# happyjin/Gaussian_process

Hardware: AMD Instinct MI355X
Metric: GP-fit+predict sec and achieved fp64 TFLOP/s, N=65536 d=8, 1/2/4/8 MI355X (higher is better)
Workload: dtype f64; 1 GPU; GP fit+predict N=65536 d=8 n_test=4096 (BASELINE configs[2]); N=65536, d=8, n_test=4096, partition=single GPU

## Files before the change

gaussian_process_amd/csrc/driver.hip:

```cpp
#include "gpmi_ctx.h"
#include "gpmi_plan.h"

namespace gpmi {

hipError_t panel_rec(hipStream_t s, double* A, int64_t ld, int64_t mrows, int64_t off, int64_t w,
                     int64_t col_offset, int64_t* info) {
    hipError_t e;
    const bool fused = tuning().panel_fused && w % 128 == 0 && off % 128 == 0;
    const int64_t leaf = fused ? 128 : IB;
    if (w <= leaf) {
        double* Ajj = A + off * ld + off;
        const int64_t below = mrows - off - leaf;
        if (fused) {
            if ((e = launch_potrf128(s, Ajj, ld, col_offset + off, info)) != hipSuccess) return e;
            if (below > 0) return launch_trsm128(s, Ajj, ld, A + (off + leaf) * ld + off, ld, below);
            return hipSuccess;
        }
        if ((e = launch_potf2_64(s, Ajj, ld, col_offset + off, info)) != hipSuccess) return e;
        if (below > 0) return launch_trsm_rlt64(s, Ajj, ld, A + (off + IB) * ld + off, ld, below);
        return hipSuccess;
    }
    const int64_t h = (w / 2) / leaf * leaf;
    if ((e = panel_rec(s, A, ld, mrows, off, h, col_offset, info)) != hipSuccess) return e;
    {
        const int64_t c0 = off + h;
        const int64_t r0 = c0 / TILE * TILE;
        const GemmArgs g = gemm_minus_lower(A + r0 * ld + c0, ld, A + r0 * ld + off, ld, A + c0 * ld + off, ld, mrows - r0,
                                            w - h, h, r0 - c0);
        if ((e = launch_gemm_nt(s, g)) != hipSuccess) return e;
    }
    return panel_rec(s, A, ld, mrows, off + h, w - h, col_offset, info);
}

hipError_t panel_factor(hipStream_t s, double* A, int64_t ld, int64_t nb, int64_t mrows,
                        int64_t col_offset, int64_t* info) {
    return panel_rec(s, A, ld, mrows, 0, nb, col_offset, info);
}

hipError_t trsm_rec(hipStream_t s, const double* L, int64_t ldl, double* X, int64_t ldx, int64_t m,
                    int64_t off, int64_t w) {
    hipError_t e;
    const bool fused = tuning().panel_fused && w % 128 == 0 && off % 128 == 0 && m % 128 == 0;
    const int64_t leaf = fused ? 128 : IB;
    if (w <= leaf) {
        if (fused) return launch_trsm128(s, L + off * ldl + off, ldl, X + off, ldx, m);
        return launch_trsm_rlt64(s, L + off * ldl + off, ldl, X + off, ldx, m);
    }
    const int64_t h = (w / 2) / leaf * leaf;
    if ((e = trsm_rec(s, L, ldl, X, ldx, m, off, h)) != hipSuccess) return e;
    const GemmArgs g = gemm_minus(X + off + h, ldx, X + off, ldx, L + (off + h) * ldl + off, ldl, m, w - h, h);
    if ((e = launch_gemm_nt(s, g)) != hipSuccess) return e;
    return trsm_rec(s, L, ldl, X, ldx, m, off + h, w - h);
}

hipError_t trsm_block(hipStream_t s, const double* L, int64_t ldl, double* X, int64_t ldx,
                      int64_t m, int64_t nb) {
    return trsm_rec(s, L, ldl, X, ldx, m, 0, nb);
}

std::vector<int64_t> block_schedule(const gpmi_ctx* c, int64_t ncols) {
    return plan_block_widths(c->block(ncols), ncols, c->nb == 0, c->ramp);
}

hipError_t cholesky_inplace(gpmi_ctx* c, double* A, int64_t ld, int64_t ncols, int64_t nrows,
                            int64_t* info, bool account, int64_t carried_rows, const SweepFollower* follow) {
    hipError_t e;
    hipStream_t sm = c->stream;
    const std::vector<int64_t> widths = block_schedule(c, ncols);
    const int64_t NB = c->block(ncols);
    const bool la = c->lookahead && c->pstream && ncols > NB && ncols >= c->la_min;
    hipStream_t sp_ = la ? c->pstream : sm;
    const bool large = la && ncols >= 49152;
    const bool slack = large && (c->slack_forms & 1);
    SharingScope shallow((la || follow) ? Sharing::beside_update().with_panel_slack(slack) : sharing());
    const bool col_on_panel = la && (!large || (c->slack_forms & 2));
    const int slot_p = account ? GPMI_T_CHOL_PANEL : GPMI_T_COUNT - 1;
    const int slot_t = account ? GPMI_T_CHOL_TRAIL : GPMI_T_COUNT - 1;
    if (la && (e = c->order(sm, sp_)) != hipSuccess) return e;
    auto trail = [&](hipStream_t st, bool counted, int64_t r0, int64_t c0, int64_t k, int64_t nb, int64_t ncol_upd) -> hipError_t {
        GemmArgs g = gemm_minus_lower(A + r0 * ld + c0, ld, A + r0 * ld + k, ld, A + c0 * ld + k, ld, nrows - r0, ncol_upd,
                                      nb, r0 - c0);
        g.role = counted ? 1 : 0;
        const GemmRoute route = gemm_nt_route(g);
        const bool dma = gemm_kernel_is_dma(route.kernel);
        size_t sp = c->span_begin(counted ? (dma ? slot_t : GPMI_T_COUNT - 1) : slot_p, st);
        hipError_t er = launch_gemm_nt(st, g, route);
        c->span_end(sp, st);
        if (account && dma && counted) {
            c->stage_ms[GPMI_T_TRAIL_LAUNCHES] += 1.0;
            c->stage_ms[GPMI_T_TRAIL_FLOPS] += gemm_nt_algorithmic_flops(g, ncols - r0 + 1 + carried_rows);
        }
        return er;
    };
    int64_t k = 0;
    hipEvent_t ev_b = nullptr;
    for (size_t step = 0; step < widths.size(); ++step) {
        const int64_t nb = widths[step];
        size_t sp = c->span_begin(slot_p, sp_);
        {
            SharingScope panel_forms(!la ? sharing().large_lds()
                                     : (ncols - k >= c->shallow_min ? Sharing::beside_update() : Sharing::chip_shared_only()).with_panel_slack(slack));
            e = panel_factor(sp_, A + k * ld + k, ld, nb, nrows - k, k, info);
        }
        c->span_end(sp, sp_);
        if (e != hipSuccess) return e;
        if (la && (e = c->order(sp_, sm)) != hipSuccess) return e;
        const int64_t r0 = k + nb;
        if (follow) {
            if ((e = c->order(sp_, follow->vs)) != hipSuccess) return e;
            {
                SharingScope solve_forms(follow->m >= 2048 ? Sharing::beside_update() : Sharing::chip_shared_only());
                if ((e = trsm_block(follow->vs, A + k * ld + k, ld, follow->V + k, follow->ldv, follow->m, nb)) != hipSuccess) return e;
            }
            if (r0 < ncols) {
                const GemmArgs g = gemm_minus(follow->V + r0, follow->ldv, follow->V + k, follow->ldv, A + r0 * ld + k, ld,
                                              follow->m, ncols - r0, nb);
                SharingScope update_forms(sharing().with_panel_slack(false));
                if ((e = launch_gemm_nt(follow->vs, g)) != hipSuccess) return e;
            }
        }
        k = r0;
        if (r0 >= ncols) continue;
        if (!la) {
            if ((e = trail(sm, true, r0, r0, r0 - nb, nb, ncols - r0)) != hipSuccess) return e;
            continue;
        }
        const int64_t nbn = widths[step + 1];
        if (!col_on_panel) {
            if ((e = trail(sm, true, r0, r0, r0 - nb, nb, nbn)) != hipSuccess) return e;
            if ((e = c->order(sm, sp_)) != hipSuccess) return e;
            if (r0 + nbn < ncols &&
                (e = trail(sm, true, r0 + nbn, r0 + nbn, r0 - nb, nb, ncols - r0 - nbn)) != hipSuccess) return e;
            continue;
        }
        if (ev_b && (e = hipStreamWaitEvent(sp_, ev_b, 0)) != hipSuccess) return e;
        if ((e = trail(sp_, false, r0, r0, r0 - nb, nb, nbn)) != hipSuccess) return e;
        if (r0 + nbn < ncols) {
            if ((e = trail(sm, true, r0 + nbn, r0 + nbn, r0 - nb, nb, ncols - r0 - nbn)) != hipSuccess) return e;
            ev_b = c->new_event();
            if (!ev_b) return c->ev_error;
            if ((e = hipEventRecord(ev_b, sm)) != hipSuccess) return e;
        }
    }
    return hipSuccess;
}

RbfArgs rbf_cross(const gpmi_ctx* c, const double* A, int64_t nA, const Box& ba, const double* B, int64_t nB, const Box& bb,
                  int64_t row0, int64_t nrows, int64_t ncols, double* out, int64_t ld) {
    RbfArgs r;
    r.A = A; r.B = B;
    r.nA = nA; r.nB = nB; r.d = c->d; r.row0 = row0; r.nrows = nrows; r.ncols = ncols;
    r.coef = c->coef; r.sig2 = c->sig2;
    r.kind = c->kind; r.kp0 = c->kp0; r.kp1 = c->kp1;
    for (int i = 0; i < 11; ++i) r.kpv[i] = c->kpv[i];
    r.diag_add = 0.; r.symmetric = 0;
// ... 224 lines not shown
```

gaussian_process_amd/csrc/gpmi_api.hip:

```cpp
#include "gpmi_ctx.h"

using namespace gpmi;

namespace gpmi {
thread_local std::string g_err;

static thread_local Tuning t_dev_tuning;
static thread_local const Tuning* t_tuning = nullptr;
const Tuning& tuning() { return t_tuning ? *t_tuning : t_dev_tuning; }
TuneScope::TuneScope(const Tuning* t) : prev(t_tuning) { t_tuning = t; }
TuneScope::~TuneScope() { t_tuning = prev; }
static thread_local Sharing t_sharing;
Sharing& sharing() { return t_sharing; }

int ard_rescale_train(gpmi_ctx* c) {
    if (!c->ard()) return GPMI_OK;
    HIP_TRY(c->Xz.ensure((size_t)c->N * c->d * 8));
    HIP_TRY(launch_scale_inputs(c->stream, c->X.as<double>(), c->ard_rdev.as<double>(), c->N, c->d, c->Xz.as<double>()));
    HIP_TRY(hipStreamSynchronize(c->stream));
    box_scale(c->boxX, c->ard_r, c->boxZ);
    return GPMI_OK;
}
int ard_rescale_test(gpmi_ctx* c) {
    if (!c->ard()) return GPMI_OK;
    HIP_TRY(c->Xsz.ensure((size_t)c->n * c->d * 8));
    HIP_TRY(launch_scale_inputs(c->stream, c->Xs.as<double>(), c->ard_rdev.as<double>(), c->n, c->d, c->Xsz.as<double>()));
    HIP_TRY(hipStreamSynchronize(c->stream));
    box_scale(c->boxXs, c->ard_r, c->boxZs);
    return GPMI_OK;
}
}

extern "C" {

int gpmi_abi_version(void) { return GPMI_ABI_VERSION; }
const char* gpmi_last_error(void) { return g_err.c_str(); }

int gpmi_device_count(int* count) {
    if (!count) return fail_arg("gpmi_device_count: null pointer");
    int n = 0;
    hipError_t e = hipGetDeviceCount(&n);
    if (e != hipSuccess) { *count = 0; return fail_runtime(e, "hipGetDeviceCount"); }
    *count = n;
    return GPMI_OK;
}

int gpmi_ctx_create(int device, gpmi_ctx** out) {
    if (!out) return fail_arg("gpmi_ctx_create: null out pointer");
    *out = nullptr;
    int n = 0;
    HIP_TRY(hipGetDeviceCount(&n));
    if (device < 0 || device >= n) return fail_arg("gpmi_ctx_create: no such device");
    HIP_TRY(hipSetDevice(device));
    gpmi_ctx* c = new gpmi_ctx();
    c->device = device;
    int prio_lo = 0, prio_hi = 0;
    (void)hipDeviceGetStreamPriorityRange(&prio_lo, &prio_hi);
    hipError_t e = hipStreamCreateWithPriority(&c->stream, hipStreamNonBlocking, prio_lo);
    if (e != hipSuccess) { delete c; return fail_runtime(e, "hipStreamCreate"); }
    e = hipStreamCreateWithPriority(&c->pstream, hipStreamNonBlocking, prio_hi);
    if (e != hipSuccess) { (void)hipStreamDestroy(c->stream); delete c; return fail_runtime(e, "hipStreamCreate"); }
    const char* env;
    if ((env = getenv("GPMI_NB"))) c->nb = std::max<int64_t>(128, atoll(env) / 128 * 128);
    if ((env = getenv("GPMI_LD_PAD"))) c->ld_pad = std::max<int64_t>(0, atoll(env) / 2 * 2);
    if ((env = getenv("GPMI_LOOKAHEAD"))) c->lookahead = atoi(env) ? 1 : 0;
    if ((env = getenv("GPMI_SLACK_FORMS"))) c->slack_forms = atoi(env) & 3;
    *out = c;
    return GPMI_OK;
}

int gpmi_ctx_destroy(gpmi_ctx* c) {
    if (!c) return GPMI_OK;
    for (gpmi_ctx* l : c->lane_ctx) (void)gpmi_ctx_destroy(l);
    c->lane_ctx.clear();
    (void)hipSetDevice(c->device);
    (void)hipStreamSynchronize(c->stream);
    for (DevBuf* b : {&c->X, &c->y, &c->A, &c->info, &c->red, &c->Xs, &c->V, &c->P, &c->vec, &c->dense,
                       &c->U, &c->Kn, &c->gpart, &c->cov_a, &c->cov_b, &c->cov_out, &c->flag, &c->vside,
                       &c->Xz, &c->Xsz, &c->ard_rdev, &c->gsum, &c->lap, &c->lap_part, &c->lap_out, &c->sm, &c->sm_part, &c->sm_E, &c->sm_B, &c->sm_out, &c->loov, &c->loow,
                       &c->sp_Zraw, &c->sp_Z, &c->sp_L, &c->sp_B, &c->sp_W, &c->sp_q, &c->sp_vec, &c->sp_part, &c->sp_scr, &c->sp_info, &c->sp_pred,
                       &c->sp_g0, &c->sp_g1, &c->sp_g2, &c->sp_gE, &c->sp_gpart, &c->sp_gvec})
        b->release();
    for (auto e : c->ev_pool) (void)hipEventDestroy(e);
    (void)hipStreamDestroy(c->stream);
    (void)hipStreamDestroy(c->pstream);
    if (c->vstream) (void)hipStreamDestroy(c->vstream);
    delete c;
    return GPMI_OK;
}

static int set_tuning_option(Tuning& t, const char* name, int64_t value) {
    if (!strcmp(name, "gemm_small_tiles")) {
        t.gemm_small_tiles = value ? 1 : 0;
    } else if (!strcmp(name, "trsm_wave")) {
        t.trsm_wave = value ? 1 : 0;
    } else if (!strcmp(name, "gemm_small_dma")) {
        t.gemm_small_dma = value ? 1 : 0;
    } else if (!strcmp(name, "gemm_persist")) {
        t.gemm_persist = value ? 1 : 0;
    } else if (!strcmp(name, "gemm_ticket")) {
        if (value < 0 || value > 2) return fail_arg("gemm_ticket must be 0 (off), 1 (trailing updates under lookahead) or 2 (every launch)");
        t.gemm_ticket = (int)value;
    } else if (!strcmp(name, "gemm_balance")) {
        t.gemm_balance = value ? 1 : 0;
    } else if (!strcmp(name, "trsv_vinv")) {
        if (value < 0 || value > 2) return fail_arg("trsv_vinv must be 0 (16 x 16 rounds), 1 (one launch per block) or 2 (one launch)");
        t.trsv_vinv = (int)value;
    } else if (!strcmp(name, "panel_fused")) {
        t.panel_fused = value ? 1 : 0;
    } else if (!strcmp(name, "rbf_blocks")) {
        if (value < 1 || value > (1 << 24)) return fail_arg("rbf_blocks must be in 1..2^24");
        t.rbf_blocks = (int)value;
    } else if (!strcmp(name, "gemm_dma_waves")) {
        if (value != 4 && value != 8) return fail_arg("gemm_dma_waves must be 4 or 8");
        t.gemm_dma_waves = (int)value;
    } else if (!strcmp(name, "gemm_tall")) {
        if (value < 0 || value > 1) return fail_arg("gemm_tall must be 0 (128 x 128 blocks) or 1 (256 x 128 blocks for large launches)");
        t.gemm_tall = (int)value;
    } else if (!strcmp(name, "tall_min_tiles")) {
        if (value < 0 || value > (1 << 30)) return fail_arg("tall_min_tiles must be in 0..2^30");
        t.tall_min_tiles = (int)value;
    } else if (!strcmp(name, "tall_min_tiles_slack")) {
        if (value < 0 || value > (1 << 30)) return fail_arg("tall_min_tiles_slack must be in 0..2^30");
        t.tall_min_tiles_slack = (int)value;
    } else if (!strcmp(name, "gemm_dma")) {
        t.gemm_use_dma = value ? 1 : 0;
    } else {
        return -1;
    }
    return GPMI_OK;
}

int gpmi_set_option(gpmi_ctx* c, const char* name, int64_t value) {
    if (!c || !name) return fail_arg("gpmi_set_option: null argument");
    if (!strcmp(name, "nb")) {
        if (value != 0 && (value < 128 || value % 128)) return fail_arg("nb must be 0 (auto) or a positive multiple of 128");
        c->nb = value;
    } else if (!strcmp(name, "ld_pad")) {
        if (value < 0 || value % 2) return fail_arg("ld_pad must be even and >= 0");
        c->ld_pad = value;
        c->res.drop_fit();
    } else if (!strcmp(name, "timing")) {
        c->timing = value ? 1 : 0;
    } else if (!strcmp(name, "lookahead")) {
        c->lookahead = value ? 1 : 0;
    } else if (!strcmp(name, "la_min")) {
        if (value < 0) return fail_arg("la_min must be >= 0");
        c->la_min = value;
    } else if (!strcmp(name, "shallow_min")) {
        if (value < 0) return fail_arg("shallow_min must be >= 0");
        c->shallow_min = value;
    } else if (!strcmp(name, "slack_forms")) {
        if (value < 0 || value > 3) return fail_arg("slack_forms: bit 0 the lower bar of the 256 x 128 form, bit 1 the next block column on the panel stream");
        c->slack_forms = (int)value;
    } else if (!strcmp(name, "one_pass_form")) {
        if (value < 0 || value > 2) return fail_arg("one_pass_form must be 0 (by size), 1 (rows ride) or 2 (rows follow)");
        c->one_pass_form = (int)value;
    } else if (!strcmp(name, "sparse_slab")) {
        if (value < 0) return fail_arg("sparse_slab must be >= 0 (0: by size)");
        c->sparse_slab = value;
    } else if (!strcmp(name, "lanes")) {
        if (value < 0 || value > 8) return fail_arg("lanes must be 0 (by size) .. 8");
        c->lanes = (int)value;
    } else if (!strcmp(name, "ramp")) {
        if (value < 0 || (value & 8) || (value >> 4) > 64) return fail_arg("ramp: bits 0-2 and a tail count of at most 64 in bits 4..");
        c->ramp = (int)value;
    } else {
        const int rc = set_tuning_option(c->tune, name, value);
        if (rc < 0) return fail_arg("gpmi_set_option: unknown option");
        return rc;
    }
    return GPMI_OK;
}

int gpmi_dev_set_option(const char* name, int64_t value) {
    if (!name) return fail_arg("gpmi_dev_set_option: null argument");
    const int rc = set_tuning_option(t_dev_tuning, name, value);
    if (rc < 0) return fail_arg("gpmi_dev_set_option: unknown option");
    return rc;
}

int gpmi_set_kernel(gpmi_ctx* c, int kind, double p0, double p1) {
    if (!c) return fail_arg("gpmi_set_kernel: null context");
    if (kind < 0 || kind == 3 || kind > 6)
        return fail_arg("gpmi_set_kernel: kind must be 0 (rbf), 1 (linear), 2 (periodic) or 4, 5, 6 (Matern nu = 1/2, 3/2, 5/2)");
    if (kind == 2 && (!(p0 != 0.0) || !(p1 != 0.0))) return fail_arg("gpmi_set_kernel: period and lengthscale must be non-zero");
    c->kind = kind; c->kp0 = p0; c->kp1 = p1;
    c->res.drop_fit();
    return GPMI_OK;
}

int gpmi_set_kernel_params(gpmi_ctx* c, int kind, const double* params, int nparams) {
    if (!c || !params) return fail_arg("gpmi_set_kernel_params: null argument");
    if (kind != 3) {
        if (kind < 0 || kind > 6 || nparams != 2) return fail_arg("gpmi_set_kernel_params: kinds 0-2 and 4-6 take 2 parameters");
        return gpmi_set_kernel(c, kind, params[0], params[1]);
    }
    if (nparams != 11) return fail_arg("gpmi_set_kernel_params: the CO2 composite kernel takes 11 hyper-parameters (CO2_example.py:86-89)");
    if (!(params[1] != 0.0) || !(params[3] != 0.0) || !(params[4] != 0.0) || !(params[6] != 0.0) || !(params[7] != 0.0) ||
        !(params[9] != 0.0))
        return fail_arg("gpmi_set_kernel_params: theta_2, 4, 5, 7, 8, 10 divide and must be non-zero");
    c->kind = 3;
    for (int i = 0; i < 11; ++i) c->kpv[i] = params[i];
    c->res.drop_fit();
    return GPMI_OK;
}

int gpmi_sync(gpmi_ctx* c) {
    if (!c) return fail_arg("gpmi_sync: null context");
    HIP_TRY(hipSetDevice(c->device));
    HIP_TRY(hipStreamSynchronize(c->stream));
    return GPMI_OK;
}

static int cov_impl(gpmi_ctx* c, int kind, const double* a, int64_t N, const double* b, int64_t M, int64_t d,
                    double p0, double p1, const double* kpv, double* out);

int gpmi_cov(gpmi_ctx* c, int kind, const double* a, int64_t N, const double* b, int64_t M, int64_t d,
             double p0, double p1, double* out) {
    if (kind < 0 || kind == 3 || kind > 6) return fail_arg("gpmi_cov: kind must be 0, 1, 2, 4, 5 or 6");
    return cov_impl(c, kind, a, N, b, M, d, p0, p1, nullptr, out);
}

int gpmi_cov_params(gpmi_ctx* c, int kind, const double* a, int64_t N, const double* b, int64_t M, int64_t d,
                    const double* params, int nparams, double* out) {
    if (!params) return fail_arg("gpmi_cov_params: null parameters");
    if (kind != 3) {
        if (kind < 0 || kind > 6 || nparams != 2) return fail_arg("gpmi_cov_params: kinds 0-2 and 4-6 take 2 parameters");
        return cov_impl(c, kind, a, N, b, M, d, params[0], params[1], nullptr, out);
    }
    if (nparams != 11) return fail_arg("gpmi_cov_params: the CO2 composite kernel takes 11 hyper-parameters");
    if (!(params[1] != 0.0) || !(params[3] != 0.0) || !(params[4] != 0.0) || !(params[6] != 0.0) || !(params[7] != 0.0) ||
        !(params[9] != 0.0))
        return fail_arg("gpmi_cov_params: theta_2, 4, 5, 7, 8, 10 divide and must be non-zero");
    return cov_impl(c, 3, a, N, b, M, d, 0., 0., params, out);
}

// ... 185 lines not shown

int gpmi_fit_predict_resident(gpmi_ctx* c, double sigma, double ell, double noise_var, double* lml, int64_t* bad_pivot,
                              double* mu, double* out2, int want_sd) {
    if (!c) return fail_arg("gpmi_fit_predict: null context");
    if (!c->res.have_test) return fail_arg("gpmi_fit_predict: no test set (call gpmi_set_test)");
    HIP_TRY(hipSetDevice(c->device));
    TuneScope tune_scope(&c->tune);
    return factorize_impl(c, sigma, ell, noise_var, lml, bad_pivot, true, mu, out2, want_sd);
}

int gpmi_fit_predict_sample_resident(gpmi_ctx* c, double sigma, double ell, double noise_var, double jitter, double* lml,
                                     int64_t* bad_pivot, double* mu, double* out2, int want_sd, double* L_out) {
    if (!c) return fail_arg("gpmi_fit_predict_sample: null context");
    if (!c->res.have_test) return fail_arg("gpmi_fit_predict_sample: no test set (call gpmi_set_test)");
    HIP_TRY(hipSetDevice(c->device));
    TuneScope tune_scope(&c->tune);
    int rc = factorize_impl(c, sigma, ell, noise_var, lml, bad_pivot, true, mu, out2, want_sd, true, jitter);
    if (rc || !L_out) return rc;
    return gpmi_post_chol(c, jitter, L_out, bad_pivot);
}

int gpmi_predict(gpmi_ctx* c, const double* Xs, int64_t n, double* mu, double* out2, int want_sd) {
    int rc = gpmi_set_test(c, Xs, n);
    if (rc) return rc;
    return gpmi_predict_resident(c, mu, out2, want_sd);
}

int gpmi_lml_grad(gpmi_ctx* c, double* d_ell, double* d_sigma) {
    if (!c || !d_ell || !d_sigma) return fail_arg("gpmi_lml_grad: null argument");
    HIP_TRY(hipSetDevice(c->device));
    const Tuning tn = resident_tuning(c);
    TuneScope tune_scope(&tn);
    return lml_grad_impl(c, d_ell, d_sigma);
}

int gpmi_lml_grad_ard(gpmi_ctx* c, double* d_r, double* d_ell, double* d_sigma, double* d_noise) {
    if (!c) return fail_arg("gpmi_lml_grad_ard: null context");
    HIP_TRY(hipSetDevice(c->device));
    const Tuning tn = resident_tuning(c);
    TuneScope tune_scope(&tn);
    return lml_grad_ard_impl(c, d_r, d_ell, d_sigma, d_noise);
}

int gpmi_loo(gpmi_ctx* c, double* mu, double* var, double* logp, double* loo) {
    if (!c) return fail_arg("gpmi_loo: null context");
    HIP_TRY(hipSetDevice(c->device));
    const Tuning tn = resident_tuning(c);
    TuneScope tune_scope(&tn);
    return loo_impl(c, mu, var, logp, loo);
}

int gpmi_loo_grad(gpmi_ctx* c, double* d_ell, double* d_sigma, double* d_noise) {
    if (!c) return fail_arg("gpmi_loo_grad: null context");
    HIP_TRY(hipSetDevice(c->device));
    const Tuning tn = resident_tuning(c);
    TuneScope tune_scope(&tn);
    return loo_grad_impl(c, d_ell, d_sigma, d_noise);
}

int gpmi_grad_trace(gpmi_ctx* c, const double* a_in, const double* b_in, int64_t N, int64_t d, double sigma,
                    double ell, const double* alpha_in, const double* Kinv_in, double* d_ell, double* d_sigma) {
    if (!c || !a_in || !b_in || !alpha_in || !Kinv_in || !d_ell || !d_sigma) return fail_arg("gpmi_grad_trace: null argument");
    HIP_TRY(hipSetDevice(c->device));
    return grad_trace_impl(c, a_in, b_in, N, d, sigma, ell, alpha_in, Kinv_in, d_ell, d_sigma);
}

int gpmi_post_chol(gpmi_ctx* c, double jitter, double* L_out, int64_t* bad_pivot) {
    if (!c || !L_out) return fail_arg("gpmi_post_chol: null argument");
    HIP_TRY(hipSetDevice(c->device));
    TuneScope tune_scope(&c->tune);
    return post_chol_impl(c, jitter, L_out, bad_pivot);
}

int gpmi_post_sample(gpmi_ctx* c, double jitter, const double* Z, int64_t num_fun, double* LZ_out, int64_t* bad_pivot) {
    if (!c || !Z || !LZ_out) return fail_arg("gpmi_post_sample: null argument");
    HIP_TRY(hipSetDevice(c->device));
    TuneScope tune_scope(&c->tune);
    return post_sample_impl(c, jitter, Z, num_fun, LZ_out, bad_pivot);
}

static int lane_prepare(gpmi_ctx* c, gpmi_ctx* l) {
    l->nb = c->nb; l->ld_pad = c->ld_pad; l->lookahead = c->lookahead; l->la_min = c->la_min; l->ramp = c->ramp; l->timing = c->timing;
    l->tune = c->tune;
    l->kind = c->kind; l->kp0 = c->kp0; l->kp1 = c->kp1;
    for (int i = 0; i < 11; ++i) l->kpv[i] = c->kpv[i];
    l->N = c->N; l->d = c->d; l->boxX = c->box_train();
    HIP_TRY(l->X.ensure((size_t)c->N * c->d * 8));
    HIP_TRY(l->y.ensure((size_t)c->N * 8));
    HIP_TRY(hipMemcpyAsync(l->X.p, c->x_train(), (size_t)c->N * c->d * 8, hipMemcpyDeviceToDevice, l->stream));
    HIP_TRY(hipMemcpyAsync(l->y.p, c->y.p, (size_t)c->N * 8, hipMemcpyDeviceToDevice, l->stream));
    HIP_TRY(hipStreamSynchronize(l->stream));
    l->res.drop_train();
    l->res.train_set();
    return GPMI_OK;
}

int gpmi_lml_batch(gpmi_ctx* c, const double* triples, int64_t T, double* lml_out, int* status_out) {
    if (!c || !triples || !lml_out) return fail_arg("gpmi_lml_batch: null argument");
    if (T < 0) return fail_arg("gpmi_lml_batch: T < 0");
    if (!c->res.have_train) return fail_arg("gpmi_lml_batch: no training set (call gpmi_set_train)");
    HIP_TRY(hipSetDevice(c->device));
    const int64_t Np = round_up(c->N, TILE);
    int L = c->lanes ? c->lanes : (Np > 32768 ? 1 : Np >= 24576 ? 3 : Np >= 12288 ? 5 : 4);
    L = (int)std::min<int64_t>(L, std::max<int64_t>(T, 1));
    struct LaMinScope {
        gpmi_ctx* c; int64_t keep;
        ~LaMinScope() { c->la_min = keep; }
    } la_scope{c, c->la_min};
    if (L > 1) c->la_min = std::max<int64_t>(c->la_min, 12288);
    while ((int)c->lane_ctx.size() < L - 1) {
        gpmi_ctx* l = nullptr;
        int rc = gpmi_ctx_create(c->device, &l);
        if (rc) return rc;
        c->lane_ctx.push_back(l);
    }
    for (int j = 0; j < L - 1; ++j) {
        int rc = lane_prepare(c, c->lane_ctx[(size_t)j]);
        if (rc) return rc;
    }
    const int parent_class = (int)((T - 1 + L) % L);
    std::vector<gpmi_ctx*> lane((size_t)L);
    for (int r = 0, nx = 0; r < L; ++r) lane[(size_t)r] = (r == parent_class) ? c : c->lane_ctx[(size_t)nx++];
    std::vector<int> lane_rc((size_t)L, GPMI_OK);
    std::vector<std::string> lane_err((size_t)L);
    std::vector<std::vector<double>> lane_ms((size_t)L, std::vector<double>(GPMI_T_COUNT, 0.0));
    auto work = [&](int r) {
        gpmi_ctx* l = lane[(size_t)r];
        TuneScope tune_scope(&l->tune);
        SharingScope shares_chip(L > 1 ? sharing().and_chip_shared() : sharing());
        if (hipSetDevice(l->device) != hipSuccess) { lane_rc[(size_t)r] = GPMI_ERR_RUNTIME; lane_err[(size_t)r] = "hipSetDevice"; return; }
        for (int64_t t = r; t < T; t += L) {
            const double ell = triples[3 * t], sigma = triples[3 * t + 1], s2 = triples[3 * t + 2];
            double lml = 0.;
            int64_t bad = 0;
            const int rc = factorize_impl(l, sigma, ell, s2, &lml, &bad);
            if (rc == GPMI_ERR_RUNTIME || rc == GPMI_ERR_BAD_ARG) {
                lane_rc[(size_t)r] = rc;
                lane_err[(size_t)r] = g_err;
                return;
            }
            lml_out[t] = lml;
            if (status_out) status_out[t] = rc;
            for (int i = 0; i < GPMI_T_COUNT; ++i) lane_ms[(size_t)r][(size_t)i] += l->stage_ms[i];
        }
    };
    if (L == 1) {
        work(0);
    } else {
        std::vector<std::thread> th;
        for (int r = 0; r < L; ++r) th.emplace_back(work, r);
        for (auto& t : th) t.join();
    }
    for (int r = 0; r < L; ++r)
        if (lane_rc[(size_t)r] != GPMI_OK) {
            g_err = lane_err[(size_t)r];
            return lane_rc[(size_t)r];
        }
    for (int i = 0; i < GPMI_T_COUNT; ++i) {
        c->stage_ms[i] = 0.0;
        for (int r = 0; r < L; ++r) c->stage_ms[i] += lane_ms[(size_t)r][(size_t)i];
    }
    return GPMI_OK;
}

int gpmi_laplace_fit(gpmi_ctx* c, double sigma, double ell, double tol, int max_iter, double* log_q, int* iters,
                     int* converged, double* f_hat) {
    if (!c) return fail_arg("gpmi_laplace_fit: null context");
    HIP_TRY(hipSetDevice(c->device));
    TuneScope tune_scope(&c->tune);
    return laplace_fit_impl(c, sigma, ell, tol, max_iter, log_q, iters, converged, f_hat);
}

int gpmi_laplace_predict_resident(gpmi_ctx* c, double* f_mean, double* f_var, double* prob) {
    if (!c) return fail_arg("gpmi_laplace_predict: null context");
    HIP_TRY(hipSetDevice(c->device));
    return laplace_predict_impl(c, f_mean, f_var, prob);
}

int gpmi_laplace_grad(gpmi_ctx* c, double* d_r, double* d_ell, double* d_sigma) {
    if (!c) return fail_arg("gpmi_laplace_grad: null context");
    HIP_TRY(hipSetDevice(c->device));
    return laplace_grad_impl(c, d_r, d_ell, d_sigma);
}

int gpmi_softmax_fit(gpmi_ctx* c, int n_classes, double sigma, double ell, double tol, int max_iter, double* log_q,
                     int* iters, int* converged, double* f_hat) {
    if (!c) return fail_arg("gpmi_softmax_fit: null context");
    HIP_TRY(hipSetDevice(c->device));
    TuneScope tune_scope(&c->tune);
    return softmax_fit_impl(c, n_classes, sigma, ell, tol, max_iter, log_q, iters, converged, f_hat);
}
// ... 48 lines not shown
```

gaussian_process_amd/csrc/gpmi_ctx.h:

```cpp
#pragma once
#include <algorithm>
#include <cmath>
#include <cstdio>
#include <cstring>
#include <limits>
#include <string>
#include <thread>
#include <vector>

#include "../../include/gpmi.h"
#include "gpmi_internal.h"
#include "gpmi_state.h"

namespace gpmi {

extern thread_local std::string g_err;

inline int fail_runtime(hipError_t e, const char* what) {
    char buf[512];
    snprintf(buf, sizeof buf, "%s: %s (hipError %d)", what, hipGetErrorString(e), (int)e);
    g_err = buf;
    return GPMI_ERR_RUNTIME;
}
inline int fail_arg(const char* what) {
    g_err = what;
    return GPMI_ERR_BAD_ARG;
}

#define HIP_TRY(expr)                                             \
    do {                                                          \
        hipError_t _e = (expr);                                   \
        if (_e != hipSuccess) return fail_runtime(_e, #expr);     \
    } while (0)

inline int64_t round_up(int64_t x, int64_t m) { return (x + m - 1) / m * m; }

struct DevBuf {
    void* p = nullptr;
    size_t cap = 0;
    hipError_t ensure(size_t bytes) {
        if (bytes <= cap) return hipSuccess;
        if (p) { hipError_t e = hipFree(p); if (e != hipSuccess) return e; p = nullptr; cap = 0; }
        hipError_t e = hipMalloc(&p, bytes);
        if (e == hipSuccess) cap = bytes;
        return e;
    }
    void release() { if (p) (void)hipFree(p); p = nullptr; cap = 0; }
    template <class T> T* as() const { return reinterpret_cast<T*>(p); }
};

struct TimedSpan { hipEvent_t a, b; int slot; };

struct Box {
    std::vector<double> lo, hi;
    bool valid = false;
    void assign(const double* X, int64_t n, int64_t d) {
        lo.assign((size_t)d, std::numeric_limits<double>::infinity());
        hi.assign((size_t)d, -std::numeric_limits<double>::infinity());
        bool finite = n > 0;
        for (int64_t i = 0; i < n; ++i)
            for (int64_t k = 0; k < d; ++k) {
                const double v = X[i * d + k];
                finite &= std::isfinite(v);
                lo[(size_t)k] = std::min(lo[(size_t)k], v);
                hi[(size_t)k] = std::max(hi[(size_t)k], v);
            }
        valid = finite;
    }
};
inline void box_scale(const Box& raw, const std::vector<double>& r, Box& out) {
    out = raw;
    if (raw.lo.size() != r.size()) { out.valid = false; return; }
    for (size_t k = 0; k < r.size(); ++k) {
        out.lo[k] = raw.lo[k] / r[k];
        out.hi[k] = raw.hi[k] / r[k];
    }
}
inline double box_max_sq(const Box& a, const Box& b) {
    if (!a.valid || !b.valid || a.lo.size() != b.lo.size()) return -1.0;
    double s = 0.0;
    for (size_t k = 0; k < a.lo.size(); ++k) {
        const double w = std::max(a.hi[k] - b.lo[k], b.hi[k] - a.lo[k]);
        s += w * w;
    }
    return std::isfinite(s) ? s : -1.0;
}

}

using gpmi::Box;
using gpmi::DevBuf;
using gpmi::TimedSpan;

struct gpmi_ctx {
    int device = 0;
    hipStream_t stream = nullptr;
    hipStream_t pstream = nullptr;
    hipStream_t vstream = nullptr;
    int64_t nb = 0;
    int64_t block(int64_t ncols) const { return nb ? nb : (ncols >= 32768 ? 2048 : ncols >= 12288 ? 1024 : 512); }
    int64_t ld_pad = 544;
    int timing = 1;
    int lookahead = 1;
    int64_t la_min = 6144;
    int64_t shallow_min = 6144;
    int slack_forms = 3;
    int one_pass_form = 0;
    int lanes = 0;
    std::vector<gpmi_ctx*> lane_ctx;
    int ramp = 0;
    gpmi::Tuning tune;
    int64_t N = 0, d = 0, Np = 0, ldA = 0, Mp = 0;
    gpmi::Resident res;
    double sig2 = 1.0, coef = -0.5;
    int kind = 0;
    double kp0 = 0., kp1 = 0.;
    double kpv[11] = {0., 0., 0., 0., 0., 0., 0., 0., 0., 0., 0.};
    DevBuf X, y, A, info, red;
    int64_t n = 0, np_ = 0, ldV = 0, ldP = 0;
    int64_t v_row0 = 0;
    double* v_rows() { return res.v_in_A ? A.as<double>() + v_row0 * ldA : V.as<double>(); }
    int64_t yrow = 0;
    double* m_row() { return A.as<double>() + yrow * ldA; }
    std::vector<double> hXs;
    Box boxX, boxXs;
    std::vector<double> ard_r;
    DevBuf Xz, Xsz, ard_rdev;
    Box boxZ, boxZs;
    bool ard() const { return !ard_r.empty(); }
    const double* x_train() const { return ard() ? Xz.as<double>() : X.as<double>(); }
    const double* x_test() const { return ard() ? Xsz.as<double>() : Xs.as<double>(); }
    const Box& box_train() const { return ard() ? boxZ : boxX; }
    const Box& box_test() const { return ard() ? boxZs : boxXs; }
    DevBuf Xs, V, P, vec, dense;
    DevBuf flag;
    DevBuf vside;
    DevBuf cov_a, cov_b, cov_out;
    DevBuf U, Kn, gpart;
    DevBuf gsum;
    double sigma = 1.0, ell = 1.0;
    double noise = 0.0;
    DevBuf loov, loow;
    DevBuf lap, lap_part, lap_out;
    int sm_classes = 0;
    DevBuf sm, sm_part, sm_E, sm_B, sm_out;
    int sp_method = 0, sp_fused = 1;
    int64_t sparse_slab = 0;
    int64_t sp_m = 0, sp_mp = 0, sp_ld = 0, sp_wrows = 0;
    Box boxU;
    DevBuf sp_Zraw, sp_Z, sp_L, sp_B, sp_W, sp_q, sp_vec, sp_part, sp_scr, sp_info, sp_pred;
    DevBuf sp_g0, sp_g1, sp_g2, sp_gE, sp_gpart, sp_gvec;
    void release_sparse_grad() {
        for (DevBuf* b : {&sp_g0, &sp_g1, &sp_g2, &sp_gE, &sp_gpart, &sp_gvec}) b->release();
    }
    std::vector<hipEvent_t> ev_pool;
    size_t ev_used = 0;
    std::vector<TimedSpan> spans;
    double stage_ms[GPMI_T_COUNT] = {0};

    hipError_t ev_error = hipSuccess;
    hipEvent_t new_event() {
        if (ev_used == ev_pool.size()) {
            hipEvent_t e = nullptr;
            const hipError_t r = hipEventCreateWithFlags(&e, hipEventDefault);
            if (r != hipSuccess) { ev_error = r; return nullptr; }
            ev_pool.push_back(e);
        }
        return ev_pool[ev_used++];
    }
    static constexpr size_t NO_SPAN = (size_t)-1;
    size_t span_begin(int slot, hipStream_t st = nullptr) {
        if (!timing) return NO_SPAN;
        TimedSpan s{new_event(), new_event(), slot};
        if (!s.a || !s.b) return NO_SPAN;
        if (hipEventRecord(s.a, st ? st : stream) != hipSuccess) return NO_SPAN;
        spans.push_back(s);
        return spans.size() - 1;
    }
    void span_end(size_t idx, hipStream_t st = nullptr) {
        if (!timing || idx == NO_SPAN) return;
        if (hipEventRecord(spans[idx].b, st ? st : stream) != hipSuccess) spans[idx].slot = GPMI_T_COUNT - 1;
    }
    hipError_t order(hipStream_t signaller, hipStream_t waiter) {
        hipEvent_t e = new_event();
        if (!e) return ev_error;
        hipError_t r = hipEventRecord(e, signaller);
        if (r != hipSuccess) return r;
        return hipStreamWaitEvent(waiter, e, 0);
    }
// ... 95 lines not shown
```

gaussian_process_amd/csrc/gpmi_plan.h:

```cpp
#pragma once
#include <math.h>
#include <stdint.h>

#include <algorithm>
#include <vector>

#if defined(__HIPCC__)
#define GPMI_HD __host__ __device__ __forceinline__
#else
#define GPMI_HD inline
#endif

namespace gpmi {

constexpr int PLAN_TILE = 128;
constexpr int DMA_MAX_SM = 128;

struct TilePlan {
    int Tm = 0, Tn = 0;
    int lower = 0;
    int64_t diag_off = 0;
    int row_block_tiles = 1;
    int S = 1, logS = 0, SM = 0, SN = 0;
    int tri = 0;
// ... 139 lines not shown
            if (!plan_tiles(q, Tm, Tn, lower, diag_off, has_row_map, row_ncols_host, row_bands, row_block_tiles, c, false, pair)) break;
            if (stairs && q.tri != 2) break;
            cand[nc] = c;
            eff[nc] = plan_xcd_efficiency(q, row_ncols_host);
            best = std::max(best, eff[nc]);
            ++nc;
        }
        for (int i = 0; i < nc; ++i)
            if (eff[i] >= best - 0.01) { force_S = cand[i]; break; }
    }
    if (force_S) S = force_S;
    for (;; S >>= 1) {
        const int SM = (p.Tm + S - 1) / S, SN = (p.Tn + S - 1) / S;
        int ns = p.tri ? SM * (SM + 1) / 2 : SM * SN;
        bool use_stairs = false;
        if (stairs && SM <= DMA_MAX_SM) {
            int tot = 0;
            p.sprefix[0] = 0;
            for (int si = 0; si < SM; ++si) {
                int64_t widest = 0;
                for (int ti = si * S; ti < std::min((si + 1) * S, p.Tm); ++ti) {
                    const int band = std::min(ti / p.row_block_tiles, row_bands - 1);
                    widest = std::max<int64_t>(widest, row_ncols_host[band]);
                }
                widest = std::max<int64_t>(widest, 0);
                const int64_t live = std::min<int64_t>(SN, (widest + (int64_t)S * PLAN_TILE - 1) / ((int64_t)S * PLAN_TILE));
                tot += (int)live;
                p.sprefix[si + 1] = tot;
            }
            ns = tot;
            use_stairs = true;
        }
        if (ns >= 32 || S == min_S || force_S) {
            p.S = S; p.SM = SM; p.SN = SN; p.nsuper = ns;
            if (use_stairs) { p.tri = 2; p.row_ncols = row_ncols_host; }
            break;
        }
    }
    p.logS = (p.S == 8) ? 3 : (p.S == 4) ? 2 : (p.S == 2) ? 1 : 0;
    p.nblocks = ((p.nsuper + 7) / 8) * 8 * ((p.S * p.S) >> p.pair);
    return true;
}

inline int64_t plan_live_tiles(int64_t Tm, int64_t Tn, int lower, int64_t diag_off, const int32_t* row_ncols_host,
                               int row_bands, int row_block_tiles) {
    int64_t n = 0;
    const int rbt = row_block_tiles > 0 ? row_block_tiles : 1;
    for (int64_t ti = 0; ti < Tm; ++ti) {
        int64_t w = Tn;
        if (lower) {
            const int64_t lim = ti * PLAN_TILE + PLAN_TILE - 1 + diag_off;
            w = lim < 0 ? 0 : std::min<int64_t>(Tn, lim / PLAN_TILE + 1);
        }
        if (row_ncols_host && row_bands > 0) {
            const int64_t nc = row_ncols_host[std::min<int64_t>(ti / rbt, row_bands - 1)];
            w = std::min<int64_t>(w, nc > 0 ? (nc + PLAN_TILE - 1) / PLAN_TILE : 0);
        }
        n += w;
    }
    return n;
}

inline std::vector<int64_t> plan_block_widths(int64_t NB, int64_t ncols, bool ramp_ok, int ramp) {
    std::vector<int64_t> w;
    if (NB <= 0 || ncols <= 0) return w;
    const bool on = ramp_ok && ramp && NB >= 1024 && ncols >= 8 * NB;
    const bool up = on && (ramp & 1), down = on && (ramp & 2);
    const int64_t tail = (ramp >> 4) ? (ramp >> 4) : 3;
    int64_t done = 0;
    while (done < ncols) {
        int64_t nb = NB;
        const int64_t left = ncols - done;
        if (up && w.size() < 2) nb = NB / 4;
        else if (up && w.size() < 3) nb = NB / 2;
        else if (down && left <= NB && (ramp & 4)) nb = NB / 4;
        else if (down && left <= tail * NB) nb = NB / 2;
        nb = std::min(nb, ncols - done);
        w.push_back(nb);
        done += nb;
    }
    return w;
}

inline double plan_tile_flops(int64_t M, int64_t N, int64_t K, int lower, int64_t diag_off) {
    if (M <= 0 || N <= 0 || K <= 0) return 0.;
    const int TN = (N % 128 == 0) ? 128 : 64;
    const int64_t Tm = M / 128, Tn = N / TN;
    int64_t tiles = 0;
    for (int64_t ti = 0; ti < Tm; ++ti) {
        if (!lower) { tiles += Tn; continue; }
        const int64_t lim = ti * 128 + 127 + diag_off;
        if (lim < 0) continue;
        const int64_t cnt = lim / TN + 1;
        tiles += cnt < Tn ? cnt : Tn;
    }
    return 2.0 * (double)tiles * 128.0 * TN * (double)K;
}

inline double plan_algorithmic_flops(int64_t M, int64_t N, int64_t K, int lower, int64_t diag_off, int64_t real_rows) {
    if (M <= 0 || N <= 0 || K <= 0) return 0.;
    const int64_t rows = std::min<int64_t>(M, real_rows);
    if (!lower) return 2.0 * (double)rows * (double)N * (double)K;
    double elems = 0.;
    const int64_t r_full = std::max<int64_t>(0, N - 1 - diag_off);
    const int64_t r_first = std::max<int64_t>(0, -diag_off);
    const int64_t tri_end = std::min(rows, r_full);
    if (tri_end > r_first) {
        const double n = (double)(tri_end - r_first);
        const double first = (double)(r_first + diag_off + 1);
        elems += n * first + n * (n - 1) / 2.0;
    }
    if (rows > r_full) elems += (double)(rows - std::max(r_full, (int64_t)0)) * (double)N;
    return 2.0 * elems * (double)K;
}

}
```

Baseline: 69.33 TFLOP/s.

## Use double-width Cholesky blocks at the front of large factorizations

Adds a wide block-width schedule that uses blocks twice (or four times) the normal width while at least wide_min columns remain, after the first block. It is on by default for large lookahead Cholesky (ncols >= 49152) and disabled for multi-lane runs. Wider blocks raise the K dimension of the trailing updates and halve the number of panel/update steps, reducing launch and synchronization overhead. In exchange the panel factorizations are larger and may be harder to hide behind the trailing update.

```diff
diff --git a/gaussian_process_amd/csrc/driver.hip b/gaussian_process_amd/csrc/driver.hip
--- a/gaussian_process_amd/csrc/driver.hip
+++ b/gaussian_process_amd/csrc/driver.hip
@@ -58,19 +58,22 @@
     return trsm_rec(s, L, ldl, X, ldx, m, 0, nb);
 }
 
-std::vector<int64_t> block_schedule(const gpmi_ctx* c, int64_t ncols) {
-    return plan_block_widths(c->block(ncols), ncols, c->nb == 0, c->ramp);
+std::vector<int64_t> block_schedule(const gpmi_ctx* c, int64_t ncols, bool slack) {
+    const int64_t NB = c->block(ncols);
+    if (c->wide_panels > 1 && (c->wide_force || (slack && c->nb == 0)))
+        return plan_block_widths_wide(NB, ncols, c->nb == 0, c->ramp, c->wide_panels, c->wide_min);
+    return plan_block_widths(NB, ncols, c->nb == 0, c->ramp);
 }
 
 hipError_t cholesky_inplace(gpmi_ctx* c, double* A, int64_t ld, int64_t ncols, int64_t nrows,
                             int64_t* info, bool account, int64_t carried_rows, const SweepFollower* follow) {
     hipError_t e;
     hipStream_t sm = c->stream;
-    const std::vector<int64_t> widths = block_schedule(c, ncols);
     const int64_t NB = c->block(ncols);
     const bool la = c->lookahead && c->pstream && ncols > NB && ncols >= c->la_min;
     hipStream_t sp_ = la ? c->pstream : sm;
     const bool large = la && ncols >= 49152;
+    const std::vector<int64_t> widths = block_schedule(c, ncols, large);
     const bool slack = large && (c->slack_forms & 1);
     SharingScope shallow((la || follow) ? Sharing::beside_update().with_panel_slack(slack) : sharing());
     const bool col_on_panel = la && (!large || (c->slack_forms & 2));
diff --git a/gaussian_process_amd/csrc/gpmi_api.hip b/gaussian_process_amd/csrc/gpmi_api.hip
--- a/gaussian_process_amd/csrc/gpmi_api.hip
+++ b/gaussian_process_amd/csrc/gpmi_api.hip
@@ -65,6 +65,8 @@
     if ((env = getenv("GPMI_LD_PAD"))) c->ld_pad = std::max<int64_t>(0, atoll(env) / 2 * 2);
     if ((env = getenv("GPMI_LOOKAHEAD"))) c->lookahead = atoi(env) ? 1 : 0;
     if ((env = getenv("GPMI_SLACK_FORMS"))) c->slack_forms = atoi(env) & 3;
+    if ((env = getenv("GPMI_WIDE_PANELS"))) { const int w = atoi(env); c->wide_panels = (w == 2 || w == 4) ? w : 0; }
+    if ((env = getenv("GPMI_WIDE_MIN"))) c->wide_min = std::max<int64_t>(0, atoll(env));
     *out = c;
     return GPMI_OK;
 }
@@ -153,6 +155,14 @@
     } else if (!strcmp(name, "slack_forms")) {
         if (value < 0 || value > 3) return fail_arg("slack_forms: bit 0 the lower bar of the 256 x 128 form, bit 1 the next block column on the panel stream");
         c->slack_forms = (int)value;
+    } else if (!strcmp(name, "wide_panels")) {
+        if (value != 0 && value != 2 && value != 4) return fail_arg("wide_panels must be 0 (uniform blocks), 2 or 4 (blocks that many times as wide at the front of a large Cholesky)");
+        c->wide_panels = (int)value;
+    } else if (!strcmp(name, "wide_min")) {
+        if (value < 0) return fail_arg("wide_min must be >= 0");
+        c->wide_min = value;
+    } else if (!strcmp(name, "wide_force")) {
+        c->wide_force = value ? 1 : 0;
     } else if (!strcmp(name, "one_pass_form")) {
         if (value < 0 || value > 2) return fail_arg("one_pass_form must be 0 (by size), 1 (rows ride) or 2 (rows follow)");
         c->one_pass_form = (int)value;
@@ -504,6 +514,7 @@
 static int lane_prepare(gpmi_ctx* c, gpmi_ctx* l) {
     l->nb = c->nb; l->ld_pad = c->ld_pad; l->lookahead = c->lookahead; l->la_min = c->la_min; l->ramp = c->ramp; l->timing = c->timing;
     l->tune = c->tune;
+    l->wide_panels = 0;
     l->kind = c->kind; l->kp0 = c->kp0; l->kp1 = c->kp1;
     for (int i = 0; i < 11; ++i) l->kpv[i] = c->kpv[i];
     l->N = c->N; l->d = c->d; l->boxX = c->box_train();
@@ -526,9 +537,10 @@
     int L = c->lanes ? c->lanes : (Np > 32768 ? 1 : Np >= 24576 ? 3 : Np >= 12288 ? 5 : 4);
     L = (int)std::min<int64_t>(L, std::max<int64_t>(T, 1));
     struct LaMinScope {
-        gpmi_ctx* c; int64_t keep;
-        ~LaMinScope() { c->la_min = keep; }
-    } la_scope{c, c->la_min};
+        gpmi_ctx* c; int64_t keep; int keep_wide;
+        ~LaMinScope() { c->la_min = keep; c->wide_panels = keep_wide; }
+    } la_scope{c, c->la_min, c->wide_panels};
+    c->wide_panels = 0;
     if (L > 1) c->la_min = std::max<int64_t>(c->la_min, 12288);
     while ((int)c->lane_ctx.size() < L - 1) {
         gpmi_ctx* l = nullptr;
diff --git a/gaussian_process_amd/csrc/gpmi_ctx.h b/gaussian_process_amd/csrc/gpmi_ctx.h
--- a/gaussian_process_amd/csrc/gpmi_ctx.h
+++ b/gaussian_process_amd/csrc/gpmi_ctx.h
@@ -105,6 +105,9 @@
     int64_t la_min = 6144;
     int64_t shallow_min = 6144;
     int slack_forms = 3;
+    int wide_panels = 2;
+    int64_t wide_min = 32768;
+    int wide_force = 0;
     int one_pass_form = 0;
     int lanes = 0;
     std::vector<gpmi_ctx*> lane_ctx;
diff --git a/gaussian_process_amd/csrc/gpmi_plan.h b/gaussian_process_amd/csrc/gpmi_plan.h
--- a/gaussian_process_amd/csrc/gpmi_plan.h
+++ b/gaussian_process_amd/csrc/gpmi_plan.h
@@ -245,6 +245,29 @@
     return w;
 }
 
+inline std::vector<int64_t> plan_block_widths_wide(int64_t NB, int64_t ncols, bool ramp_ok, int ramp, int wide, int64_t wide_min) {
+    std::vector<int64_t> w;
+    if (NB <= 0 || ncols <= 0) return w;
+    const bool on = ramp_ok && ramp && NB >= 1024 && ncols >= 8 * NB;
+    const bool up = on && (ramp & 1), down = on && (ramp & 2);
+    const int64_t tail = (ramp >> 4) ? (ramp >> 4) : 3;
+    const int64_t WB = wide > 1 ? (int64_t)wide * NB : NB;
+    int64_t done = 0;
+    while (done < ncols) {
+        int64_t nb = NB;
+        const int64_t left = ncols - done;
+        if (up && w.size() < 2) nb = NB / 4;
+        else if (up && w.size() < 3) nb = NB / 2;
+        else if (down && left <= NB && (ramp & 4)) nb = NB / 4;
+        else if (down && left <= tail * NB) nb = NB / 2;
+        else if (!w.empty() && left >= wide_min && left >= WB) nb = WB;
+        nb = std::min(nb, ncols - done);
+        w.push_back(nb);
+        done += nb;
+    }
+    return w;
+}
+
 inline double plan_tile_flops(int64_t M, int64_t N, int64_t K, int lower, int64_t diag_off) {
     if (M <= 0 || N <= 0 || K <= 0) return 0.;
     const int TN = (N % 128 == 0) ? 128 : 64;
```

New measurement: 69.99 TFLOP/s (median of 6 runs). Within noise of the previous version (+0.9%).
